# facebookresearch/theseus

Hardware: NVIDIA H100
Metric: LM iterations/sec on batched SE3 pose-graph (2500 poses, global batch 2048 over N GPUs, LM + block-sparse Cholesky, fp64) (higher is better)
Workload: dtype f64

## Files before the change

theseus_b200/csrc/thb_front.cu:

```cuda
#include <stdlib.h>

#include "thb_common.cuh"

namespace thb {

#ifdef THB_SIMT_EMU
#define THB_PDL_TRIGGER() do { } while (0)
#define THB_PDL_WAIT() do { } while (0)
#define FRONT_LAUNCH(K, grid, block, smem, cs, arg) K<<<grid, block, smem, cs>>>(arg)
#else
#define THB_PDL_TRIGGER() asm volatile("griddepcontrol.launch_dependents;" ::: "memory")
#define THB_PDL_WAIT() asm volatile("griddepcontrol.wait;" ::: "memory")
#define FRONT_LAUNCH(K, grid, block, smem, cs, arg) thb::front_launch_pdl(K, grid, block, smem, cs, arg)
static inline bool front_pdl_enabled() {
  static const bool on = [] { const char* e = getenv("THB_FRONT_PDL"); return e != nullptr && e[0] == '1'; }();
  return on;
}
template <typename A>
static inline void front_launch_pdl(void (*kernel)(A), dim3 grid, dim3 block, size_t smem, cudaStream_t cs, const A& arg) {
  cudaLaunchConfig_t cfg = {};
  cfg.gridDim = grid; cfg.blockDim = block; cfg.dynamicSmemBytes = smem; cfg.stream = cs;
  cudaLaunchAttribute at[1];
  at[0].id = cudaLaunchAttributeProgrammaticStreamSerialization;
  at[0].val.programmaticStreamSerializationAllowed = 1;
  cfg.attrs = at; cfg.numAttrs = front_pdl_enabled() ? 1 : 0;
  cudaLaunchKernelEx(&cfg, kernel, arg);
}
#endif

#ifdef THB_SIMT_EMU
__device__ inline void front_mma884(double& c0, double& c1, double a, double b) {
  const int lane = threadIdx.x & 31, lr = lane >> 2, lc = lane & 3;
  for (int k = 0; k < 4; k++) {
    const double av = __shfl_sync(0xffffffffu, a, lr * 4 + k);
    const double b0 = __shfl_sync(0xffffffffu, b, (2 * lc) * 4 + k);
    const double b1 = __shfl_sync(0xffffffffu, b, (2 * lc + 1) * 4 + k);
    c0 += av * b0;
    c1 += av * b1;
  }
}
#else
__device__ __forceinline__ void front_mma884(double& c0, double& c1, double a, double b) {
  asm volatile("mma.sync.aligned.m8n8k4.row.col.f64.f64.f64.f64 {%0,%1}, {%2}, {%3}, {%0,%1};\n" : "+d"(c0), "+d"(c1) : "d"(a), "d"(b));
}
#endif

__host__ __device__ __forceinline__ int front_pad_ld(int x) { return ((x + 11) / 16) * 16 + 4; }

struct FrontArgs {
  thb_front_plan p;
  int s0;
  int64_t B;
  double* factor;
  const double* alpha;
  const double* beta;
  double* arena_cur;
  const double* arena_child;
  int32_t* info;
  int prefetch;
  const double* ata;
  int64_t ata_stride;
  const double* rhs;
  double* work;
  double* v_cur;
  const double* v_child;
};

__device__ __forceinline__ double front_panel_in(const FrontArgs& a, const double* Lg, int64_t poff, int64_t item, int64_t e) {
  if (a.ata == nullptr) return Lg[e];
  const int32_t m = a.p.pmap[poff + e];
  return m >= 0 ? a.ata[item * a.ata_stride + m] : 0.0;
}

constexpr int FRONT_WD_LD = 20;
#ifndef FRONT_PL
#define FRONT_PL 4
#endif
constexpr int FRONT_MAX_CHILDREN = 8;

__host__ __device__ __forceinline__ int64_t front_smem_doubles(int w, int b, int nchildren) {
  const int b16 = (b + 15) & ~15, w8 = (w + 7) & ~7;
  return (int64_t)(w8 + b16 + 8) * front_pad_ld(w8) + 8 * FRONT_WD_LD + 3 * FRONT_MAX_CHILDREN
         + ((int64_t)nchildren * (w + b) + 1) / 2 + 2;
}

__device__ __forceinline__ int front_leaf8(double* __restrict__ T, int ld, double* __restrict__ Wd, int lane) {
  const int ln = lane < 8 ? lane : 0;
  double row[8];
#pragma unroll
  for (int q = 0; q < 8; q++) row[q] = T[ln * ld + q];
  int fail = 0;
  double invd = 0.0;
#pragma unroll
  for (int c = 0; c < 8; c++) {
    const double d = __shfl_sync(0xffffffffu, row[c], c);
    if (!(d > 0.0) && fail == 0) fail = c + 1;
    double inv = rsqrt(d);
    inv = inv * (1.5 - 0.5 * d * inv * inv);
    const double sq = d * inv;
    if (lane == c) invd = inv;
    const double lrc = (lane == c) ? sq : row[c] * inv;
    row[c] = lrc;
#pragma unroll
    for (int q = c + 1; q < 8; q++) {
      const double lqc = __shfl_sync(0xffffffffu, lrc, q);
      row[q] -= lrc * lqc;
    }
  }
  if (lane < 8) {
#pragma unroll
    for (int q = 0; q < 8; q++)
      if (q <= lane) T[lane * ld + q] = row[q];
  }
  double x[8];
#pragma unroll
  for (int rr = 0; rr < 8; rr++) {
    double sacc = (lane == rr) ? 1.0 : 0.0;
#pragma unroll
    for (int k = 0; k < rr; k++) {
      const double lrk = __shfl_sync(0xffffffffu, row[k], rr);
      sacc -= lrk * x[k];
    }
    x[rr] = sacc * __shfl_sync(0xffffffffu, invd, rr);
  }
  if (lane < 8) {
#pragma unroll
    for (int rr = 0; rr < 8; rr++) Wd[rr * FRONT_WD_LD + lane] = (rr >= lane) ? x[rr] : 0.0;
  }
  return fail;
}

__device__ __forceinline__ void front_diag_block(double* PN, int ldp, int jb, double* Wd, int lane, int w, int first, int32_t* info) {
  const int lr = lane >> 2, lc = lane & 3;
  double c0 = 0.0, c1 = 0.0;
  const double* Arow = PN + (8 * jb + lr) * ldp + lc;
  for (int k = 0; k < 8 * jb; k += 4) {
    const double av = Arow[k];
    front_mma884(c0, c1, av, av);
  }
  double* d = PN + (8 * jb + lr) * ldp + 8 * jb + 2 * lc;
  d[0] -= c0;
  d[1] -= c1;
  __syncwarp();
  const int fail = front_leaf8(PN + (8 * jb) * ldp + 8 * jb, ldp, Wd, lane);
  if (lane == 0 && fail != 0 && 8 * jb + fail <= w) atomicCAS(info, 0, first + 8 * jb + fail);
}

template <bool TWO>
__device__ __forceinline__ void front_tile_column(double* PN, int ldp, int jb, int rt0, const double* Wd, int lane) {
  const int lr = lane >> 2, lc = lane & 3;
  double x00 = 0.0, x01 = 0.0, x10 = 0.0, x11 = 0.0;
  const double* A0 = PN + (8 * rt0 + lr) * ldp + lc;
  const double* Bj = PN + (8 * jb + lr) * ldp + lc;
  for (int k = 0; k < 8 * jb; k += 4) {
    const double bf = Bj[k];
    front_mma884(x00, x01, A0[k], bf);
    if (TWO) front_mma884(x10, x11, A0[8 * ldp + k], bf);
  }
  double* X0 = PN + (8 * rt0 + lr) * ldp + 8 * jb + 2 * lc;
  X0[0] -= x00; X0[1] -= x01;
  if (TWO) { X0[8 * ldp] -= x10; X0[8 * ldp + 1] -= x11; }
  __syncwarp();
  x00 = x01 = x10 = x11 = 0.0;
#pragma unroll
  for (int k = 0; k < 8; k += 4) {
    const double bf = Wd[lr * FRONT_WD_LD + k + lc];
    front_mma884(x00, x01, A0[8 * jb + k], bf);
    if (TWO) front_mma884(x10, x11, A0[8 * ldp + 8 * jb + k], bf);
  }
  __syncwarp();
  X0[0] = x00; X0[1] = x01;
  if (TWO) { X0[8 * ldp] = x10; X0[8 * ldp + 1] = x11; }
}

struct FrontChild {
  const double* src;
  int ldg, lo, hi, uoff;
};

__device__ __forceinline__ double front_warp_trsv_lower(const double* T, int ld, double ui, int cw, int lane) {
  const double rd = lane < cw ? 1.0 / T[lane * ld + lane] : 0.0;
  for (int k = 0; k < cw; k++) {
    const double yk = __shfl_sync(0xffffffffu, ui * rd, k);
    if (lane == k) ui = yk;
    else if (lane > k && lane < cw) ui -= T[lane * ld + k] * yk;
  }
  return ui;
}

struct FrontRowsGlobal {
  static constexpr bool kInPanel = false;
  const double* L;
  int w;
  double* T;
  __device__ __forceinline__ const double* row(int i) const { return L + (int64_t)i * w; }
  __device__ __forceinline__ const double* diag(int k0, int cw, int tid, int nthreads, int* ld) const {
    for (int e = tid; e < cw * cw; e += nthreads) {
      const int i = e / cw, j = e - i * cw;
      T[i * 33 + j] = L[(int64_t)(k0 + i) * w + k0 + j];
    }
    *ld = 33;
    return T;
  }
};
struct FrontRowsPanel {
  static constexpr bool kInPanel = true;
  const double* PN;
  int ldp, w, shift;
  __device__ __forceinline__ const double* row(int i) const { return PN + (i < w ? i : i + shift) * ldp; }
  __device__ __forceinline__ const double* diag(int k0, int, int, int, int* ld) const {
    *ld = ldp;
    return PN + k0 * ldp + k0;
  }
};

template <int THREADS, typename Rows>
__device__ __forceinline__ void front_forward_elim(const Rows& R, double* u, int us, int w, int r, int tid, int lane) {
  for (int k0 = 0; k0 < w; k0 += 32) {
    const int cw = min(32, w - k0);
    int ld;
    const double* T = R.diag(k0, cw, tid, THREADS, &ld);
    __syncthreads();
    if (tid < 32) {
      const double ui = front_warp_trsv_lower(T, ld, lane < cw ? u[(k0 + lane) * us] : 0.0, cw, lane);
      if (lane < cw) u[(k0 + lane) * us] = ui;
    }
    __syncthreads();
    for (int i = k0 + cw + tid; i < r; i += THREADS) {
      const double* row = R.row(i) + k0;
      double s = 0.0;
      if constexpr (Rows::kInPanel) {
#pragma unroll 2
        for (int k = 0; k < cw; k++) s += row[k] * u[(k0 + k) * us];
      } else {
        for (int k = 0; k < cw; k++) s += row[k] * u[(k0 + k) * us];
      }
      u[i * us] -= s;
    }
    __syncthreads();
  }
}

template <int THREADS>
__global__ void __launch_bounds__(THREADS, 1024 / THREADS) front_small_kernel(FrontArgs a) {
  extern __shared__ double sm[];
  const thb_front_plan& p = a.p;
  const int tid = threadIdx.x, lane = tid & 31, warp = tid >> 5;
  constexpr int NW = THREADS / 32;
  const int lr = lane >> 2, lc = lane & 3;
  const int64_t item = blockIdx.x;
  THB_PDL_TRIGGER();
  const int64_t* FD = p.fd + (int64_t)(a.s0 + blockIdx.y) * 8;
  const int t = (int)FD[0];
  const int w = (int)FD[1], b = (int)FD[2], r = w + b;
  const int f_first = (int)FD[3];
  const int64_t f_panel_off = FD[4], f_cb_off = FD[5];
  const int f_cb_ld = (int)FD[6];
  const int c_begin = (int)(FD[7] & 0xffffffffLL);
  const int nch = min((int)(FD[7] >> 32), FRONT_MAX_CHILDREN);
  const int b16 = (b + 15) & ~15, w8 = (w + 7) & ~7;
  const int ldp = front_pad_ld(w8);
  const int prow = w8 + b16 + 8;
  double* PN = sm;
  double* Wd = PN + prow * ldp;
  FrontChild* ch = reinterpret_cast<FrontChild*>(Wd + 8 * FRONT_WD_LD);
  int32_t* INV = reinterpret_cast<int32_t*>(Wd + 8 * FRONT_WD_LD + 3 * FRONT_MAX_CHILDREN);
  for (int q = 0; q < nch; q++) {
    const int64_t* PC = p.pc + (int64_t)(c_begin + q) * 6;
    const double* csrc = a.arena_child + item * p.arena_size + PC[0];
    const int cld = (int)(PC[1] & 0xffffffffLL), cbc = (int)(PC[1] >> 32);
    if (tid == 0) {
      ch[q].src = csrc;
      ch[q].ldg = cld;
      ch[q].lo = (int)PC[2];
      ch[q].hi = (int)PC[3];
      ch[q].uoff = (int)PC[5];
    }
    const int32_t* inv = p.c_inv + PC[4];
    for (int l = tid; l < r; l += THREADS) INV[q * r + l] = inv[l];
    (void)cbc;
  }
  for (int e = tid; e < prow * ldp; e += THREADS) sm[e] = 0.0;
  THB_PDL_WAIT();
#ifndef THB_SIMT_EMU
  if (a.rhs != nullptr) {
    for (int i = tid; i < w; i += THREADS) asm volatile("prefetch.global.L2 [%0];\n" ::"l"(a.rhs + item * p.n + p.perm[f_first + i]));
    for (int q = 0; q < nch; q++) {
      const int64_t* PC = p.pc + (int64_t)(c_begin + q) * 6;
      const double* cu = a.v_child + item * p.varena_size + PC[5];
      for (int off = tid * 16; off < (int)(PC[1] >> 32); off += THREADS * 16) asm volatile("prefetch.global.L2 [%0];\n" ::"l"(cu + off));
    }
  }
  for (int q = 0; a.prefetch != 0 && q < nch; q++) {
    const int64_t* PC = p.pc + (int64_t)(c_begin + q) * 6;
    const double* csrc = a.arena_child + item * p.arena_size + PC[0];
    const int cld = (int)(PC[1] & 0xffffffffLL), cbc = (int)(PC[1] >> 32);
    for (int off = tid * 16; off < cbc * cld; off += THREADS * 16) {
      const int i = off / cld, j = off - i * cld;
      if (j <= i) asm volatile("prefetch.global.L2 [%0];\n" ::"l"(csrc + off));
    }
  }
#endif
  __syncthreads();
  if (tid < w8 - w) PN[(w + tid) * ldp + w + tid] = 1.0;
  double* Lg = a.factor + item * p.data_size + f_panel_off;
  {
    const double al = a.alpha != nullptr ? a.alpha[item] : 0.0;
    const double be = a.beta != nullptr ? a.beta[item] : 0.0;
    const int total = r * w;
    for (int e0 = tid; e0 < total; e0 += FRONT_PL * THREADS) {
      int ii[FRONT_PL], jj[FRONT_PL];
      double v[FRONT_PL];
#pragma unroll
      for (int u = 0; u < FRONT_PL; u++) {
        const int e = e0 + u * THREADS;
        ii[u] = e / w;
        jj[u] = e - ii[u] * w;
        if (e >= total || jj[u] > ii[u]) ii[u] = -1;
        v[u] = ii[u] >= 0 ? front_panel_in(a, Lg, f_panel_off, item, e) : 0.0;
      }
#pragma unroll
      for (int u = 0; u < FRONT_PL; u++)
        if (ii[u] >= 0 && ii[u] == jj[u]) v[u] = v[u] + (al * v[u] + be);
      for (int q = 0; q < nch; q++) {
        const double* src = ch[q].src;
        const int ldg = ch[q].ldg, lo = ch[q].lo, hi = ch[q].hi;
        const int32_t* inv = INV + q * r;
#pragma unroll
        for (int u = 0; u < FRONT_PL; u++) {
          if (ii[u] >= lo && jj[u] <= hi) {
            const int ci = inv[ii[u]], cj = inv[jj[u]];
            if (ci >= 0 && cj >= 0) v[u] += src[(int64_t)ci * ldg + cj];
          }
        }
      }
#pragma unroll
      for (int u = 0; u < FRONT_PL; u++)
        if (ii[u] >= 0) PN[(ii[u] < w ? ii[u] : ii[u] + (w8 - w)) * ldp + jj[u]] = v[u];
    }
  }
  double* U = PN + w8;
  if (a.rhs != nullptr) {
    for (int i = tid; i < r; i += THREADS) {
      double v = i < w ? a.rhs[item * p.n + p.perm[f_first + i]] : 0.0;
      for (int q = 0; q < nch; q++) {
        if (i >= ch[q].lo && i <= ch[q].hi) {
          const int k = INV[q * r + i];
          if (k >= 0) v += a.v_child[item * p.varena_size + ch[q].uoff + k];
        }
      }
      U[i * ldp] = v;
    }
  }
  __syncthreads();
  const int nbk = w8 / 8, nrt = (w8 + b16) / 8;
  for (int jb = 0; jb < nbk; jb++) {
    if (warp == 0) front_diag_block(PN, ldp, jb, Wd, lane, w, f_first, a.info + item);
    __syncthreads();
    const int npair = (nrt - jb) / 2;
    for (int q = warp; q < npair; q += NW) front_tile_column<true>(PN, ldp, jb, jb + 1 + 2 * q, Wd, lane);
    __syncthreads();
  }
  {
    int i = tid / w, j = tid - i * w;
    const int di = THREADS / w, dj = THREADS - di * w;
    for (int e = tid; e < r * w; e += THREADS) {
      Lg[e] = (j > i) ? 0.0 : PN[(i < w ? i : i + (w8 - w)) * ldp + j];
      i += di; j += dj;
      if (j >= w) { j -= w; i++; }
    }
  }
  if (a.rhs != nullptr) {
    front_forward_elim<THREADS>(FrontRowsPanel{PN, ldp, w, w8 - w}, U, ldp, w, r, tid, lane);
    for (int i = tid; i < w; i += THREADS) a.work[item * p.n + f_first + i] = U[i * ldp];
    double* ub = a.v_cur + item * p.varena_size + p.f_u_off[t];
    for (int i = tid; i < b; i += THREADS) ub[i] = U[(w + i) * ldp];
  }
  if (b == 0) return;
  double* dst = a.arena_cur + item * p.arena_size + f_cb_off;
  const int ldg_out = f_cb_ld;
  const double* P = PN + w8 * ldp;
  const int nmt = b16 / 16, ntl = nmt * (nmt + 1) / 2;
  for (int q = warp; q < ntl; q += NW) {
    int R = (int)((sqrtf(8.0f * (float)q + 1.0f) - 1.0f) * 0.5f);
    while ((R + 1) * (R + 2) / 2 <= q) R++;
    while (R * (R + 1) / 2 > q) R--;
    const int ct = q - R * (R + 1) / 2;
    double gch[2][2][2] = {{{0.0, 0.0}, {0.0, 0.0}}, {{0.0, 0.0}, {0.0, 0.0}}};
    const int li0 = w + 16 * R + lr, lj0 = w + 16 * ct + 2 * lc;
    for (int qc = 0; qc < nch; qc++) {
      if (w + 16 * R + 15 >= ch[qc].lo && w + 16 * ct <= ch[qc].hi) {
        const int32_t* inv = INV + qc * r;
        const double* src = ch[qc].src;
        const int ldg = ch[qc].ldg;
        int ci[2], cj[2][2];
#pragma unroll
        for (int mi = 0; mi < 2; mi++) ci[mi] = (li0 + 8 * mi < r) ? inv[li0 + 8 * mi] : -1;
#pragma unroll
        for (int ni = 0; ni < 2; ni++)
#pragma unroll
          for (int u = 0; u < 2; u++) cj[ni][u] = (lj0 + 8 * ni + u < r) ? inv[lj0 + 8 * ni + u] : -1;
#pragma unroll
        for (int mi = 0; mi < 2; mi++)
#pragma unroll
          for (int ni = 0; ni < 2; ni++)
#pragma unroll
            for (int u = 0; u < 2; u++)
              if (ci[mi] >= 0 && cj[ni][u] >= 0 && cj[ni][u] <= ci[mi]) gch[mi][ni][u] += src[(int64_t)ci[mi] * ldg + cj[ni][u]];
      }
    }
    double acc[2][2][2] = {{{0.0, 0.0}, {0.0, 0.0}}, {{0.0, 0.0}, {0.0, 0.0}}};
    const double* Pa = P + (16 * R + lr) * ldp + lc;
    const double* Pb = P + (16 * ct + lr) * ldp + lc;
    for (int k4 = 0; k4 < w8; k4 += 4) {
      const double a0 = Pa[k4], a1 = Pa[8 * ldp + k4];
      const double b0 = Pb[k4], b1 = Pb[8 * ldp + k4];
      front_mma884(acc[0][0][0], acc[0][0][1], a0, b0);
      front_mma884(acc[0][1][0], acc[0][1][1], a0, b1);
      front_mma884(acc[1][0][0], acc[1][0][1], a1, b0);
      front_mma884(acc[1][1][0], acc[1][1][1], a1, b1);
    }
#pragma unroll
    for (int mi = 0; mi < 2; mi++)
#pragma unroll
      for (int ni = 0; ni < 2; ni++) {
        acc[mi][ni][0] = gch[mi][ni][0] - acc[mi][ni][0];
        acc[mi][ni][1] = gch[mi][ni][1] - acc[mi][ni][1];
      }
#pragma unroll
    for (int mi = 0; mi < 2; mi++) {
      const int i = 16 * R + 8 * mi + lr;
      if (i < b) {
        double* drow = dst + (int64_t)i * ldg_out;
#pragma unroll
        for (int ni = 0; ni < 2; ni++)
#pragma unroll
          for (int u = 0; u < 2; u++) {
            const int jj = 16 * ct + 8 * ni + 2 * lc + u;
            if (jj <= i) drow[jj] = acc[mi][ni][u];
          }
      }
    }
  }
}

constexpr int ASM_ROWS = 16, ASM_THREADS = 256;

__device__ __forceinline__ int front_map_big(int l, int w, int wpad) { return l < w ? l : wpad + (l - w); }

__global__ void __launch_bounds__(ASM_THREADS) front_assemble_kernel(FrontArgs a, int t) {
  extern __shared__ double sm[];
  const thb_front_plan& p = a.p;
  const int tid = threadIdx.x;
  const int64_t item = blockIdx.x;
  const int w = p.f_w[t], b = p.f_b[t], r = w + b, wpad = p.f_wpad[t], np = p.f_np[t];
  const int R0 = blockIdx.y * ASM_ROWS;
  const int nc = min(np, 128 * (R0 / 128 + 1));
  const int c_first = p.child_ptr[t], n_children = p.child_ptr[t + 1] - c_first;
  if (n_children <= FRONT_MAX_CHILDREN) {
    const double* Lgg = a.factor + item * p.data_size + p.f_panel_off[t];
    const double alg = a.alpha != nullptr ? a.alpha[item] : 0.0;
    const double beg = a.beta != nullptr ? a.beta[item] : 0.0;
    double* Fg = a.arena_cur + item * p.arena_size + p.f_fr_off[t] + (int64_t)R0 * np;
    __shared__ const double* s_src[FRONT_MAX_CHILDREN];
    __shared__ const int32_t* s_inv[FRONT_MAX_CHILDREN];
    __shared__ int s_ld[FRONT_MAX_CHILDREN];
    if (tid < n_children) {
      const int c = p.child_list[c_first + tid];
      s_src[tid] = a.arena_child + item * p.arena_size + p.f_cb_off[c];
      s_inv[tid] = p.c_inv + p.c_inv_ptr[c];
      s_ld[tid] = p.f_cb_ld[c];
    }
    __syncthreads();
    const int64_t poff = p.f_panel_off[t];
    const int total = ASM_ROWS * nc;
    for (int e0 = tid; e0 < total; e0 += 4 * ASM_THREADS) {
      int li[4], lj[4];
      double v[4];
#pragma unroll
      for (int u = 0; u < 4; u++) {
        const int e = e0 + u * ASM_THREADS;
        const int rr = e / nc, fc = e - rr * nc;
        const int fr = R0 + rr;
        li[u] = fr < w ? fr : ((fr >= wpad && fr - wpad + w < r) ? fr - wpad + w : -1);
        lj[u] = fc < w ? fc : ((fc >= wpad && fc - wpad + w < r) ? fc - wpad + w : -1);
        v[u] = 0.0;
        if (e >= total) {
          li[u] = lj[u] = -2;
        } else if (li[u] < 0 || lj[u] < 0) {
          v[u] = (fr == fc) ? 1.0 : 0.0;
          li[u] = -1;
        } else if (lj[u] > li[u]) {
          li[u] = -1;
        } else if (lj[u] < w) {
          v[u] = front_panel_in(a, Lgg, poff, item, (int64_t)li[u] * w + lj[u]);
        }
      }
#pragma unroll
      for (int u = 0; u < 4; u++)
        if (li[u] >= 0 && li[u] == lj[u] && lj[u] < w) v[u] = v[u] + (alg * v[u] + beg);
      for (int q = 0; q < n_children; q++) {
        const double* src = s_src[q];
        const int32_t* inv = s_inv[q];
        const int ldg = s_ld[q];
        int ci[4], cj[4];
#pragma unroll
        for (int u = 0; u < 4; u++) {
          ci[u] = li[u] >= 0 ? inv[li[u]] : -1;
          cj[u] = li[u] >= 0 ? inv[lj[u]] : -1;
        }
#pragma unroll
        for (int u = 0; u < 4; u++)
          if (ci[u] >= 0 && cj[u] >= 0) v[u] += src[(int64_t)ci[u] * ldg + cj[u]];
      }
#pragma unroll
      for (int u = 0; u < 4; u++) {
        const int e = e0 + u * ASM_THREADS;
        if (e < total) Fg[e + (int64_t)(e / nc) * (np - nc)] = v[u];
      }
    }
    return;
  }
  double* buf = sm;
  for (int e = tid; e < ASM_ROWS * nc; e += ASM_THREADS) buf[e] = 0.0;
  __syncthreads();
  const double* Lg = a.factor + item * p.data_size + p.f_panel_off[t];
  const double al = a.alpha != nullptr ? a.alpha[item] : 0.0;
  const double be = a.beta != nullptr ? a.beta[item] : 0.0;
  const int wlim = min(wpad, nc);
  for (int e = tid; e < ASM_ROWS * wlim; e += ASM_THREADS) {
    const int rr = e / wlim, j = e - rr * wlim;
    const int fr = R0 + rr;
    int i = -1;
    if (fr < w) i = fr;
    else if (fr >= wpad && fr - wpad + w < r) i = fr - wpad + w;
    if (i >= 0) {
      if (j < w && !(i < w && j > i)) {
        double v = front_panel_in(a, Lg, p.f_panel_off[t], item, (int64_t)i * w + j);
        if (i == j) v = v + (al * v + be);
        buf[rr * nc + j] = v;
      }
    } else if (j == fr) {
      buf[rr * nc + j] = 1.0;
    }
  }
  for (int rr = tid; rr < ASM_ROWS; rr += ASM_THREADS) {
    const int fr = R0 + rr;
    if (fr >= wpad + b) buf[rr * nc + fr] = 1.0;
  }
  __syncthreads();
  for (int ci = p.child_ptr[t]; ci < p.child_ptr[t + 1]; ci++) {
    const int c = p.child_list[ci];
    const int bc = p.f_b[c], ldg = p.f_cb_ld[c];
    const int32_t* rel = p.f_rel + p.rel_ptr[c];
    int lo = 0, hi = bc;
    while (lo < hi) { const int mid = (lo + hi) >> 1; if (front_map_big(rel[mid], w, wpad) < R0) lo = mid + 1; else hi = mid; }
    const int i0 = lo;
    hi = bc;
    while (lo < hi) { const int mid = (lo + hi) >> 1; if (front_map_big(rel[mid], w, wpad) < R0 + ASM_ROWS) lo = mid + 1; else hi = mid; }
    const int i1 = lo;
    if (i1 > i0) {
      const double* src = a.arena_child + item * p.arena_size + p.f_cb_off[c];
      for (int i = i0 + (tid >> 5); i < i1; i += ASM_THREADS / 32) {
        const int fr = front_map_big(rel[i], w, wpad) - R0;
        const double* srow = src + (int64_t)i * ldg;
        for (int j = tid & 31; j <= i; j += 32) buf[fr * nc + front_map_big(rel[j], w, wpad)] += srow[j];
      }
      __syncthreads();
    }
  }
  double* F = a.arena_cur + item * p.arena_size + p.f_fr_off[t] + (int64_t)R0 * np;
  for (int e = tid; e < ASM_ROWS * nc; e += ASM_THREADS) {
    const int rr = e / nc, c = e - rr * nc;
    F[(int64_t)rr * np + c] = buf[e];
  }
}

__global__ void __launch_bounds__(256) front_extract_kernel(FrontArgs a, int t) {
  const thb_front_plan& p = a.p;
  const int64_t item = blockIdx.x;
  const int w = p.f_w[t], b = p.f_b[t], r = w + b, wpad = p.f_wpad[t], np = p.f_np[t];
  const double* F = a.arena_cur + item * p.arena_size + p.f_fr_off[t];
  double* Lg = a.factor + item * p.data_size + p.f_panel_off[t];
  for (int e = blockIdx.y * blockDim.x + threadIdx.x; e < r * w; e += gridDim.y * blockDim.x) {
    const int i = e / w, j = e - i * w;
    const int fr = i < w ? i : wpad + (i - w);
    Lg[e] = (i < w && j > i) ? 0.0 : F[(int64_t)fr * np + j];
  }
}

struct FrontSolveArgs {
  thb_front_plan p;
  int s0;
  int64_t B;
  const double* factor;
  const double* rhs;
  double* x;
  double* work;
  double* v_cur;
  const double* v_child;
  int stage_doubles;
};

__device__ __forceinline__ double front_warp_trsv_upper(const double* T, double ti, int cw, int lane) {
  const double rd = lane < cw ? 1.0 / T[lane * 33 + lane] : 0.0;
  for (int k = cw - 1; k >= 0; k--) {
    const double xk = __shfl_sync(0xffffffffu, ti * rd, k);
    if (lane == k) ti = xk;
    else if (lane < k) ti -= T[k * 33 + lane] * xk;
  }
  return ti;
}

template <int THREADS>
__global__ void __launch_bounds__(THREADS) front_forward_kernel(FrontSolveArgs a) {
  extern __shared__ double sm[];
  const thb_front_plan& p = a.p;
  const int tid = threadIdx.x, lane = tid & 31;
  const int64_t item = blockIdx.x;
  THB_PDL_TRIGGER();
  const int64_t* FD = p.fd + (int64_t)(a.s0 + blockIdx.y) * 8;
  const int t = (int)FD[0];
  const int w = (int)FD[1], b = (int)FD[2], r = w + b, first = (int)FD[3];
  THB_PDL_WAIT();
  double* u = sm;
  double* T = sm + ((r + 1) & ~1);
  const double* Lg = a.factor + item * p.data_size + FD[4];
  if (r * w <= a.stage_doubles) {
    double* Ls = T + 32 * 33 + 1 + (THREADS & ~1) + 2;
    for (int e = tid; e < r * w; e += THREADS) Ls[e] = Lg[e];
    Lg = Ls;
  }
  {
    const int c0 = (int)(FD[7] & 0xffffffffLL), nchild = (int)(FD[7] >> 32);
    for (int i = tid; i < r; i += THREADS) {
      double v = i < w ? a.rhs[item * p.n + p.perm[first + i]] : 0.0;
      for (int q = 0; q < nchild; q++) {
        const int64_t* PC = p.pc + (int64_t)(c0 + q) * 6;
        if (i >= (int)PC[2] && i <= (int)PC[3]) {
          const int k = p.c_inv[PC[4] + i];
          if (k >= 0) v += a.v_child[item * p.varena_size + PC[5] + k];
        }
      }
      u[i] = v;
    }
  }
  __syncthreads();
  front_forward_elim<THREADS>(FrontRowsGlobal{Lg, w, T}, u, 1, w, r, tid, lane);
  for (int i = tid; i < w; i += THREADS) a.work[item * p.n + first + i] = u[i];
  if (b > 0) {
    double* ub = a.v_cur + item * p.varena_size + p.f_u_off[t];
    for (int i = tid; i < b; i += THREADS) ub[i] = u[w + i];
  }
}

template <int THREADS>
__global__ void __launch_bounds__(THREADS) front_backward_kernel(FrontSolveArgs a) {
  extern __shared__ double sm[];
  const thb_front_plan& p = a.p;
  const int tid = threadIdx.x, lane = tid & 31, warp = tid >> 5;
  const int64_t item = blockIdx.x;
  THB_PDL_TRIGGER();
  const int64_t* FD = p.fd + (int64_t)(a.s0 + blockIdx.y) * 8;
  const int t = (int)FD[0];
  const int w = (int)FD[1], b = (int)FD[2], r = w + b, first = (int)FD[3];
  THB_PDL_WAIT();
  double* xf = sm;
  double* T = sm + ((r + 1) & ~1);
  double* part = T + 32 * 33 + 1;
  const double* Lg = a.factor + item * p.data_size + FD[4];
  if (r * w <= a.stage_doubles) {
    double* Ls = T + 32 * 33 + 1 + (THREADS & ~1) + 2;
    for (int e = tid; e < r * w; e += THREADS) Ls[e] = Lg[e];
    Lg = Ls;
  }
  double* wk = a.work + item * p.n;
  const int32_t* rows = p.f_rows + p.rows_ptr[t];
  for (int i = tid; i < r; i += THREADS) xf[i] = i < w ? wk[first + i] : wk[rows[i - w]];
  __syncthreads();
  const int nchunk = (w + 31) / 32;
  for (int ch = nchunk - 1; ch >= 0; ch--) {
    const int k0 = ch * 32, cw = min(32, w - k0);
    const int RG = THREADS / cw;
    const int kk = tid % cw, rg = tid / cw;
    for (int e = tid; e < cw * cw; e += THREADS) {
      const int i = e / cw, j = e - i * cw;
      T[i * 33 + j] = Lg[(int64_t)(k0 + i) * w + k0 + j];
    }
    double acc = 0.0;
    if (rg < RG) {
      const double* col = Lg + k0 + kk;
      int i = k0 + cw + rg;
      for (; i + 3 * RG < r; i += 4 * RG) {
        const double l0 = col[(int64_t)i * w], l1 = col[(int64_t)(i + RG) * w], l2 = col[(int64_t)(i + 2 * RG) * w],
                     l3 = col[(int64_t)(i + 3 * RG) * w];
        acc += l0 * xf[i];
        acc += l1 * xf[i + RG];
        acc += l2 * xf[i + 2 * RG];
        acc += l3 * xf[i + 3 * RG];
      }
      for (; i < r; i += RG) acc += col[(int64_t)i * w] * xf[i];
    }
    part[tid] = acc;
    __syncthreads();
    if (warp == 0) {
      double tk = 0.0;
      if (lane < cw) {
        tk = xf[k0 + lane];
        for (int g = 0; g < RG; g++) tk -= part[g * cw + lane];
      }
      tk = front_warp_trsv_upper(T, tk, cw, lane);
      if (lane < cw) xf[k0 + lane] = tk;
    }
    __syncthreads();
  }
  for (int i = tid; i < w; i += THREADS) {
    const double v = xf[i];
    wk[first + i] = v;
    a.x[item * p.n + p.perm[first + i]] = v;
  }
}

static inline int front_threads_of_class(int cls) { return cls == 0 ? 64 : (cls == 1 ? 128 : 256); }

template <typename K>
static inline int front_set_smem(K kernel, size_t bytes, size_t* cache) {
  if (bytes > *cache) {
    cudaError_t e = cudaFuncSetAttribute(kernel, cudaFuncAttributeMaxDynamicSharedMemorySize, (int)bytes);
    if (e != cudaSuccess) return (int)e;
    *cache = bytes;
  }
  return 0;
}

static int front_solve_launch(const thb_front_plan* p, const int64_t* L, int pass, const double* factor, const double* rhs, double* x,
                              double* work, double* varena, int64_t B, cudaStream_t cs) {
  static size_t fw_set[3] = {0, 0, 0}, bw_set[3] = {0, 0, 0};
  static const int64_t stage_cap = [] { const char* e = getenv("THB_SOLVE_STAGE"); return e != nullptr ? (int64_t)atoll(e) : (int64_t)0; }();
  const int depth = (int)L[0], cls = (int)L[1], begin = (int)L[2], count = (int)L[3];
  FrontSolveArgs a;
  a.p = *p; a.s0 = begin; a.B = B; a.factor = factor; a.rhs = rhs; a.x = x; a.work = work;
  a.v_cur = varena != nullptr ? varena + (int64_t)(depth & 1) * B * p->varena_size : nullptr;
  a.v_child = varena != nullptr ? varena + (int64_t)((depth + 1) & 1) * B * p->varena_size : nullptr;
  const int kc = cls > 2 ? 2 : cls;
  const int threads = front_threads_of_class(kc);
  const int64_t r_max = L[5];
  const int64_t stage = (cls < 3 && L[6] > 0) ? (L[6] < stage_cap ? L[6] : stage_cap) : 0;
  a.stage_doubles = (int)stage;
  const size_t smem = (size_t)(((r_max + 1) & ~1LL) + 32 * 33 + 1 + threads + 2 + stage + 2) * 8;
  const dim3 grid((unsigned)B, (unsigned)count);
  if (pass == 0) {
    if (kc == 0) { int rc = front_set_smem(front_forward_kernel<64>, smem, &fw_set[0]); if (rc) return rc;
                   FRONT_LAUNCH(front_forward_kernel<64>, grid, 64, smem, cs, a); }
    else if (kc == 1) { int rc = front_set_smem(front_forward_kernel<128>, smem, &fw_set[1]); if (rc) return rc;
                        FRONT_LAUNCH(front_forward_kernel<128>, grid, 128, smem, cs, a); }
    else { int rc = front_set_smem(front_forward_kernel<256>, smem, &fw_set[2]); if (rc) return rc;
           FRONT_LAUNCH(front_forward_kernel<256>, grid, 256, smem, cs, a); }
  } else {
    if (kc == 0) { int rc = front_set_smem(front_backward_kernel<64>, smem, &bw_set[0]); if (rc) return rc;
                   FRONT_LAUNCH(front_backward_kernel<64>, grid, 64, smem, cs, a); }
    else if (kc == 1) { int rc = front_set_smem(front_backward_kernel<128>, smem, &bw_set[1]); if (rc) return rc;
                        FRONT_LAUNCH(front_backward_kernel<128>, grid, 128, smem, cs, a); }
    else { int rc = front_set_smem(front_backward_kernel<256>, smem, &bw_set[2]); if (rc) return rc;
           FRONT_LAUNCH(front_backward_kernel<256>, grid, 256, smem, cs, a); }
  }
  THB_CHECK_LAUNCH();
  return THB_OK;
}

static int front_factor(const thb_front_plan* p, const int64_t* launches, int64_t num_launches, double* factor, const double* ata,
                        int64_t ata_stride, const double* alpha, const double* beta, double* arena, void* dense_ws, int64_t dense_ws_bytes,
                        int32_t* info, const double* rhs, double* work, double* varena, int64_t B, thb_stream_t stream) {
  if (p == nullptr || launches == nullptr || factor == nullptr || arena == nullptr || info == nullptr || B < 0) return THB_ERR_BAD_ARG;
  if (B == 0 || p->S == 0) return THB_OK;
  if (B > 65535LL * 32768LL) return THB_ERR_UNSUPPORTED;
  cudaStream_t cs = thb_cs(stream);
  THB_CUDA(cudaMemsetAsync(info, 0, (size_t)B * 4, cs));
  static size_t smem_set[5] = {0, 0, 0, 0, 0}, asm_set = 0;
  static const int thr_cls[2] = {[] { const char* e = getenv("THB_FRONT_T0"); const int v = e ? atoi(e) : 64; return (v == 128 || v == 256) ? v : 64; }(),
                                 [] { const char* e = getenv("THB_FRONT_T1"); const int v = e ? atoi(e) : 128; return v == 256 ? 256 : 128; }()};
  static int front_prefetch_flag = -1;
  if (front_prefetch_flag < 0) {
    const char* e = getenv("THB_FRONT_PREFETCH");
    front_prefetch_flag = (e != nullptr && e[0] == '1') ? 1 : 0;
  }
  static const int fuse_max = [] { const char* e = getenv("THB_FRONT_FUSE_MAX"); return e != nullptr ? atoi(e) : 1024; }();
  for (int64_t l = 0; l < num_launches; l++) {
    const int64_t* L = launches + l * THB_FRONT_LAUNCH_COLS;
    const int depth = (int)L[0], cls = (int)L[1], begin = (int)L[2], count = (int)L[3];
    FrontArgs a;
    a.p = *p; a.s0 = begin; a.B = B; a.factor = factor; a.alpha = alpha; a.beta = beta; a.info = info;
    a.ata = (ata != nullptr && p->pmap != nullptr) ? ata : nullptr; a.ata_stride = ata_stride;
    a.prefetch = front_prefetch_flag;
    a.arena_cur = arena + (int64_t)(depth & 1) * B * p->arena_size;
    a.arena_child = arena + (int64_t)((depth + 1) & 1) * B * p->arena_size;
    a.rhs = rhs; a.work = work;
    a.v_cur = rhs != nullptr ? varena + (int64_t)(depth & 1) * B * p->varena_size : nullptr;
    a.v_child = rhs != nullptr ? varena + (int64_t)((depth + 1) & 1) * B * p->varena_size : nullptr;
    if (cls < 3) {
      const size_t smem = (size_t)L[4];
#ifndef THB_SIMT_EMU
      if (smem > 227 * 1024) return THB_ERR_UNSUPPORTED;
#endif
      const dim3 grid((unsigned)B, (unsigned)count);
      if (count > 65535) return THB_ERR_UNSUPPORTED;
      const int threads = (cls == 0 && thr_cls[0] == 64) ? 64
                          : ((cls == 0 && thr_cls[0] == 128) || (cls == 1 && thr_cls[1] == 128)) ? 128
                          : (cls <= 1 || smem <= 56 * 1024) ? 256 : (smem <= 113 * 1024 ? 512 : 1024);
      const bool fused = rhs != nullptr && threads <= fuse_max;
      if (!fused) a.rhs = nullptr;
      if (threads == 64) {
        int rc = front_set_smem(front_small_kernel<64>, smem, &smem_set[0]); if (rc) return rc;
        FRONT_LAUNCH(front_small_kernel<64>, grid, 64, smem, cs, a);
      } else if (threads == 128) {
        int rc = front_set_smem(front_small_kernel<128>, smem, &smem_set[1]); if (rc) return rc;
        FRONT_LAUNCH(front_small_kernel<128>, grid, 128, smem, cs, a);
      } else if (threads == 256) {
        int rc = front_set_smem(front_small_kernel<256>, smem, &smem_set[2]); if (rc) return rc;
        FRONT_LAUNCH(front_small_kernel<256>, grid, 256, smem, cs, a);
      } else if (threads == 512) {
        int rc = front_set_smem(front_small_kernel<512>, smem, &smem_set[3]); if (rc) return rc;
        FRONT_LAUNCH(front_small_kernel<512>, grid, 512, smem, cs, a);
      } else {
        int rc = front_set_smem(front_small_kernel<1024>, smem, &smem_set[4]); if (rc) return rc;
        FRONT_LAUNCH(front_small_kernel<1024>, grid, 1024, smem, cs, a);
      }
      THB_CHECK_LAUNCH();
      if (rhs != nullptr && !fused) {
        const int rc = front_solve_launch(p, L, 0, factor, rhs, nullptr, work, varena, B, cs);
        if (rc != THB_OK) return rc;
      }
    } else {
      const int64_t np = L[5], nb_piv = L[6], fr_off = L[7], first = L[8];
      const int t = (int)L[9];
#ifdef THB_SIMT_EMU
      (void)np; (void)nb_piv; (void)fr_off; (void)first; (void)t; (void)dense_ws; (void)dense_ws_bytes; (void)asm_set;
      return THB_ERR_UNSUPPORTED;
#else
      if (dense_ws == nullptr || np % 128 != 0 || np > 8192) return THB_ERR_BAD_ARG;
      const size_t smem = (size_t)ASM_ROWS * np * 8;
      int rc = front_set_smem(front_assemble_kernel, smem, &asm_set); if (rc) return rc;
      front_assemble_kernel<<<dim3((unsigned)B, (unsigned)(np / ASM_ROWS)), ASM_THREADS, smem, cs>>>(a, t);
      THB_CHECK_LAUNCH();
      rc = thb_potrf_partial_inplace_f64(a.arena_cur + fr_off, p->arena_size, np, (int32_t)nb_piv, (int32_t)L[10], (int32_t)(nb_piv * 64 + L[11]),
                                         (int32_t)first, info, B, dense_ws, dense_ws_bytes, stream);
      if (rc != THB_OK) return rc;
      front_extract_kernel<<<dim3((unsigned)B, 8), 256, 0, cs>>>(a, t);
      THB_CHECK_LAUNCH();
      if (rhs != nullptr) {
        rc = front_solve_launch(p, L, 0, factor, rhs, nullptr, work, varena, B, cs);
        if (rc != THB_OK) return rc;
      }
#endif
    }
  }
  return THB_OK;
}

}

extern "C" {

int64_t thb_front_small_smem_bytes(int32_t w, int32_t b, int32_t nchildren) { return thb::front_smem_doubles(w, b, nchildren) * 8; }

int thb_front_factor_f64(const thb_front_plan* p, const int64_t* launches, int64_t num_launches, double* factor, const double* ata,
                         int64_t ata_stride, const double* alpha, const double* beta, double* arena, void* dense_ws, int64_t dense_ws_bytes,
                         int32_t* info, int64_t B, thb_stream_t stream) {
  return thb::front_factor(p, launches, num_launches, factor, ata, ata_stride, alpha, beta, arena, dense_ws, dense_ws_bytes, info, nullptr,
                           nullptr, nullptr, B, stream);
}

int thb_front_factor_forward_f64(const thb_front_plan* p, const int64_t* launches, int64_t num_launches, double* factor, const double* ata,
                                 int64_t ata_stride, const double* alpha, const double* beta, double* arena, void* dense_ws,
                                 int64_t dense_ws_bytes, int32_t* info, const double* rhs, double* work, double* varena, int64_t B,
                                 thb_stream_t stream) {
  if (rhs == nullptr || work == nullptr || varena == nullptr) return THB_ERR_BAD_ARG;
  return thb::front_factor(p, launches, num_launches, factor, ata, ata_stride, alpha, beta, arena, dense_ws, dense_ws_bytes, info, rhs, work,
                           varena, B, stream);
}

int thb_front_solve_f64(const thb_front_plan* p, const int64_t* launches, int64_t num_launches, const double* factor, const double* rhs,
                        double* x, double* work, double* varena, int64_t B, thb_stream_t stream) {
  if (p == nullptr || launches == nullptr || factor == nullptr || rhs == nullptr || x == nullptr || work == nullptr || varena == nullptr ||
      B < 0)
    return THB_ERR_BAD_ARG;
  if (B == 0 || p->S == 0) return THB_OK;
  const int rc = thb_front_forward_f64(p, launches, num_launches, factor, rhs, work, varena, B, stream);
  if (rc != THB_OK) return rc;
  return thb_front_backward_f64(p, launches, num_launches, factor, x, work, B, stream);
}

int thb_front_forward_f64(const thb_front_plan* p, const int64_t* launches, int64_t num_launches, const double* factor, const double* rhs,
                          double* work, double* varena, int64_t B, thb_stream_t stream) {
  if (p == nullptr || launches == nullptr || factor == nullptr || rhs == nullptr || work == nullptr || varena == nullptr || B < 0)
    return THB_ERR_BAD_ARG;
  if (B == 0 || p->S == 0) return THB_OK;
  cudaStream_t cs = thb_cs(stream);
  for (int64_t q = 0; q < num_launches; q++) {
    const int rc = thb::front_solve_launch(p, launches + q * THB_FRONT_LAUNCH_COLS, 0, factor, rhs, nullptr, work, varena, B, cs);
    if (rc != THB_OK) return rc;
  }
  return THB_OK;
}

int thb_front_backward_f64(const thb_front_plan* p, const int64_t* launches, int64_t num_launches, const double* factor, double* x,
                           double* work, int64_t B, thb_stream_t stream) {
  if (p == nullptr || launches == nullptr || factor == nullptr || x == nullptr || work == nullptr || B < 0) return THB_ERR_BAD_ARG;
  if (B == 0 || p->S == 0) return THB_OK;
  cudaStream_t cs = thb_cs(stream);
  for (int64_t q = num_launches - 1; q >= 0; q--) {
    const int rc = thb::front_solve_launch(p, launches + q * THB_FRONT_LAUNCH_COLS, 1, factor, nullptr, x, work, nullptr, B, cs);
    if (rc != THB_OK) return rc;
  }
  return THB_OK;
}

}
```

Before: 4.997.

## Overlap forward elimination with panel store and use dynamic tile scheduling

In the small front kernel, a subset of warps now runs the forward triangular elimination on a named barrier while the remaining warps write the factor panel to global memory at the same time. The update-tile loop takes tiles from a shared atomic counter instead of a static stride per warp, and the panel dot product is skewed per lane group to spread shared-memory bank accesses. This is meant to hide the global store latency and even out warp load, at the cost of extra atomics and fewer threads working on the elimination.

```diff
diff --git a/theseus_b200/csrc/thb_front.cu b/theseus_b200/csrc/thb_front.cu
--- a/theseus_b200/csrc/thb_front.cu
+++ b/theseus_b200/csrc/thb_front.cu
@@ -214,32 +214,67 @@
   }
 };
 
-template <int THREADS, typename Rows>
+template <int GROUP, bool WHOLE_CTA>
+__device__ __forceinline__ void front_group_sync() {
+#ifdef THB_SIMT_EMU
+  static_assert(WHOLE_CTA, "the host emulation has no named barriers");
+  __syncthreads();
+#else
+  if constexpr (WHOLE_CTA) __syncthreads();
+  else asm volatile("bar.sync 1, %0;" ::"n"(GROUP) : "memory");
+#endif
+}
+
+template <int GROUP, bool WHOLE_CTA, typename Rows>
 __device__ __forceinline__ void front_forward_elim(const Rows& R, double* u, int us, int w, int r, int tid, int lane) {
   for (int k0 = 0; k0 < w; k0 += 32) {
     const int cw = min(32, w - k0);
     int ld;
-    const double* T = R.diag(k0, cw, tid, THREADS, &ld);
-    __syncthreads();
+    const double* T = R.diag(k0, cw, tid, GROUP, &ld);
+    front_group_sync<GROUP, WHOLE_CTA>();
     if (tid < 32) {
       const double ui = front_warp_trsv_lower(T, ld, lane < cw ? u[(k0 + lane) * us] : 0.0, cw, lane);
       if (lane < cw) u[(k0 + lane) * us] = ui;
     }
-    __syncthreads();
-    for (int i = k0 + cw + tid; i < r; i += THREADS) {
+    front_group_sync<GROUP, WHOLE_CTA>();
+    for (int i = k0 + cw + tid; i < r; i += GROUP) {
       const double* row = R.row(i) + k0;
       double s = 0.0;
       if constexpr (Rows::kInPanel) {
+        const int skew = (lane >> 2) & 3;
 #pragma unroll 2
-        for (int k = 0; k < cw; k++) s += row[k] * u[(k0 + k) * us];
+        for (int kk = 0; kk < cw + 3; kk++) {
+          const int k = kk - skew;
+          if ((unsigned)k < (unsigned)cw) s += row[k] * u[(k0 + k) * us];
+        }
       } else {
         for (int k = 0; k < cw; k++) s += row[k] * u[(k0 + k) * us];
       }
       u[i * us] -= s;
     }
-    __syncthreads();
-  }
-}
+    front_group_sync<GROUP, WHOLE_CTA>();
+  }
+}
+
+__device__ __forceinline__ void front_store_panel(double* __restrict__ Lg, const double* __restrict__ PN, int ldp, int w, int w8, int r, int tid,
+                                                  int nthreads) {
+  int i = tid / w, j = tid - i * w;
+  const int di = nthreads / w, dj = nthreads - di * w;
+  for (int e = tid; e < r * w; e += nthreads) {
+    Lg[e] = (j > i) ? 0.0 : PN[(i < w ? i : i + (w8 - w)) * ldp + j];
+    i += di; j += dj;
+    if (j >= w) { j -= w; i++; }
+  }
+}
+
+__device__ __forceinline__ void front_store_forward(const FrontArgs& a, const double* U, int ldp, int64_t item, int t, int f_first, int w, int b,
+                                                    int tid, int nthreads) {
+  for (int i = tid; i < w; i += nthreads) a.work[item * a.p.n + f_first + i] = U[i * ldp];
+  double* ub = a.v_cur + item * a.p.varena_size + a.p.f_u_off[t];
+  for (int i = tid; i < b; i += nthreads) ub[i] = U[(w + i) * ldp];
+}
+
+__host__ __device__ constexpr int front_elim_warps(int threads) { return threads >= 256 ? 4 : threads / 64; }
 
 template <int THREADS>
 __global__ void __launch_bounds__(THREADS, 1024 / THREADS) front_small_kernel(FrontArgs a) {
@@ -254,8 +289,7 @@
   const int t = (int)FD[0];
   const int w = (int)FD[1], b = (int)FD[2], r = w + b;
   const int f_first = (int)FD[3];
-  const int64_t f_panel_off = FD[4], f_cb_off = FD[5];
-  const int f_cb_ld = (int)FD[6];
+  const int64_t f_panel_off = FD[4];
   const int c_begin = (int)(FD[7] & 0xffffffffLL);
   const int nch = min((int)(FD[7] >> 32), FRONT_MAX_CHILDREN);
   const int b16 = (b + 15) & ~15, w8 = (w + 7) & ~7;
@@ -281,6 +315,8 @@
     (void)cbc;
   }
   for (int e = tid; e < prow * ldp; e += THREADS) sm[e] = 0.0;
+  int* next_tile = reinterpret_cast<int*>(Wd + 8);
+  if (tid == 0) *next_tile = 0;
   THB_PDL_WAIT();
 #ifndef THB_SIMT_EMU
   if (a.rhs != nullptr) {
@@ -361,30 +397,35 @@
     for (int q = warp; q < npair; q += NW) front_tile_column<true>(PN, ldp, jb, jb + 1 + 2 * q, Wd, lane);
     __syncthreads();
   }
-  {
-    int i = tid / w, j = tid - i * w;
-    const int di = THREADS / w, dj = THREADS - di * w;
-    for (int e = tid; e < r * w; e += THREADS) {
-      Lg[e] = (j > i) ? 0.0 : PN[(i < w ? i : i + (w8 - w)) * ldp + j];
-      i += di; j += dj;
-      if (j >= w) { j -= w; i++; }
-    }
-  }
+#ifdef THB_SIMT_EMU
+  front_store_panel(Lg, PN, ldp, w, w8, r, tid, THREADS);
   if (a.rhs != nullptr) {
-    front_forward_elim<THREADS>(FrontRowsPanel{PN, ldp, w, w8 - w}, U, ldp, w, r, tid, lane);
-    for (int i = tid; i < w; i += THREADS) a.work[item * p.n + f_first + i] = U[i * ldp];
-    double* ub = a.v_cur + item * p.varena_size + p.f_u_off[t];
-    for (int i = tid; i < b; i += THREADS) ub[i] = U[(w + i) * ldp];
-  }
+    front_forward_elim<THREADS, true>(FrontRowsPanel{PN, ldp, w, w8 - w}, U, ldp, w, r, tid, lane);
+    front_store_forward(a, U, ldp, item, t, f_first, w, b, tid, THREADS);
+  }
+#else
+  constexpr int NE = front_elim_warps(THREADS);
+  if (a.rhs != nullptr && warp < NE) {
+    front_forward_elim<32 * NE, false>(FrontRowsPanel{PN, ldp, w, w8 - w}, U, ldp, w, r, tid, lane);
+    front_store_forward(a, U, ldp, item, t, f_first, w, b, tid, 32 * NE);
+  } else {
+    const int t0 = a.rhs != nullptr ? 32 * NE : 0;
+    front_store_panel(Lg, PN, ldp, w, w8, r, tid - t0, THREADS - t0);
+  }
+#endif
   if (b == 0) return;
-  double* dst = a.arena_cur + item * p.arena_size + f_cb_off;
-  const int ldg_out = f_cb_ld;
+  double* dst = a.arena_cur + item * p.arena_size + FD[5];
+  const int ldg_out = (int)FD[6];
   const double* P = PN + w8 * ldp;
-  const int nmt = b16 / 16, ntl = nmt * (nmt + 1) / 2;
-  for (int q = warp; q < ntl; q += NW) {
+  const int nmt = b16 / 16;
+  for (;;) {
+    int q = 0;
+    if (lane == 0) q = atomicAdd(next_tile, 1);
+    q = __shfl_sync(0xffffffffu, q, 0);
     int R = (int)((sqrtf(8.0f * (float)q + 1.0f) - 1.0f) * 0.5f);
     while ((R + 1) * (R + 2) / 2 <= q) R++;
     while (R * (R + 1) / 2 > q) R--;
+    if (R >= nmt) break;
     const int ct = q - R * (R + 1) / 2;
     double gch[2][2][2] = {{{0.0, 0.0}, {0.0, 0.0}}, {{0.0, 0.0}, {0.0, 0.0}}};
     const int li0 = w + 16 * R + lr, lj0 = w + 16 * ct + 2 * lc;
@@ -646,7 +687,7 @@
     }
   }
   __syncthreads();
-  front_forward_elim<THREADS>(FrontRowsGlobal{Lg, w, T}, u, 1, w, r, tid, lane);
+  front_forward_elim<THREADS, true>(FrontRowsGlobal{Lg, w, T}, u, 1, w, r, tid, lane);
   for (int i = tid; i < w; i += THREADS) a.work[item * p.n + first + i] = u[i];
   if (b > 0) {
     double* ub = a.v_cur + item * p.varena_size + p.f_u_off[t];
```

Result: faster. 5.182, median of 6 (+3.7%).
